# AndreiBarsan/DynSLAM

Hardware: AMD Instinct MI355X
Metric: frames/sec TSDF integrate+raycast (KITTI 1242x375, 5mm voxels); HBM GB/s vs peak (higher is better)
Workload: dtype f32; 1 GPU; configs[1]: static map only, synthetic KITTI-like street 1242x375, preset 5mm (voxel 0.005 m, mu 0.02 m), frames 5..2062 of a 2063-frame sequence, one volume per GPU; visible_blocks_last_frame=122661, allocated_blocks=8388608, status=3, decay=False, swap=False, instances=0

## Files before the change

### __graft_entry__.py

```python
import os
import subprocess
import sys

ROOT = os.path.dirname(os.path.abspath(__file__))
CSRC = os.path.join(ROOT, "dynslam_amd", "csrc")
HIP_LIB = os.path.join(CSRC, "libdsr_hip.so")
HIP_SOURCES = ["dsr_engine.hip", "dsr_view.hip", "dsr_exchange.hip", "dsr_hostio.hip", "dsr_profile.hip", "dsr_track.hip",
               "dsr_eval.hip", "dsr_snapshot.hip", "dsr_merge.hip"]
HIP_HEADERS = ["dsr_internal.h", "dsr_device.h", "k_alloc.h", "k_small.h", "k_batch.h", "k_composite.h", "k_decay.h", "k_edges.h", "k_integrate.h",
               "k_raycast.h", "k_swap.h", "k_mesh.h", "mc_tables.h", "k_track.h", "k_batch_track.h", "dsr_math.h", "k_eval.h",
               "k_batch_gc.h", "k_snapshot.h", "k_mesh_complete.h", "k_merge.h"]
HIPCC_COMPILE_FLAGS = ["--offload-arch=gfx950", "-O3", "-std=c++17", "-fPIC", "-ffp-contract=off", "-fno-slp-vectorize",
                       "-fno-fast-math", "-Wall", "-Wno-unused-function"]
HIPCC_FLAGS = HIPCC_COMPILE_FLAGS + ["-shared"]


def _stale(target, deps):
    if not os.path.exists(target):
        return True
    t = os.path.getmtime(target)
    return any(os.path.getmtime(d) > t for d in deps)


def build_hip(force=False):
    srcs = [os.path.join(CSRC, s) for s in HIP_SOURCES]
    deps = srcs + [os.path.join(CSRC, h) for h in HIP_HEADERS] + [os.path.join(ROOT, "include", h) for h in ("dsr.h", "dsr_track.h", "dsr_eval.h", "dsr_gc.h", "dsr_snapshot.h", "dsr_mesh.h")]
# ... 97 lines not shown
```

### dynslam_amd/csrc/dsr_engine.hip

```cpp
#include <sched.h>

#include "dsr_internal.h"
#include "dsr_math.h"
using namespace dsr_internal;
#include "k_alloc.h"
#include "k_composite.h"
#include "k_decay.h"
#include "k_integrate.h"
#include "k_raycast.h"
#include "k_swap.h"
#include "k_mesh.h"
#include "k_mesh_complete.h"
#include "k_small.h"
#include "k_batch.h"
#include "k_batch_gc.h"
#include "../../include/dsr_track.h"
#include "../../include/dsr_gc.h"
#include "../../include/dsr_mesh.h"

extern "C" {
int dsri_batch_flush(dsr_batch *b);
bool dsri_batch_is_live(dsr_batch *b);
void dsri_batch_drop_deferred(dsr_batch *b);
}

namespace dsr_internal {
std::atomic<int> g_enginesOnDevice[64];
}
// ... 22 lines not shown
bool m4_inv(const Mat4 &in, Mat4 &out) { return dsr_math::m4_inv(in.m, out.m); }

}


namespace {

void prof_resolve(dsr_engine *e) {
  if (e->profPending.empty()) return;
  if (e->viewStream) (void)hipStreamSynchronize(e->viewStream);
  (void)hipStreamSynchronize(e->stream);
  if (e->sideStream) (void)hipStreamSynchronize(e->sideStream);
  if (e->device >= 0 && e->device < 64 && g_ioStream[e->device]) (void)hipStreamSynchronize(g_ioStream[e->device]);
  for (auto &p : e->profPending) {
    float ms = 0.0f;
    if (hipEventElapsedTime(&ms, p.a, p.b) == hipSuccess) { e->profRecs[p.rec].ms += ms; e->profRecs[p.rec].launches++; }
    e->eventPool.push_back(p.a); e->eventPool.push_back(p.b);
  }
  e->profPending.clear();
}

FrameP make_frame_params(const dsr_engine *e, const Mat4 &M, const Mat4 &invM, const float proj[4]) {
  FrameP p;
  memset(&p, 0, sizeof p);
  p.M = M; p.invM = invM;
  p.M_rgb = m4_mul(e->calibInv, M);
  p.proj = make_float4(proj[0], proj[1], proj[2], proj[3]);
  p.proj_rgb = make_float4(e->calib.rgb.fx, e->calib.rgb.fy, e->calib.rgb.cx, e->calib.rgb.cy);
  p.mu = e->s.mu; p.voxelSize = e->s.voxel_size;
  p.vfMin = e->s.view_frustum_min; p.vfMax = e->s.view_frustum_max;
  p.W = e->W; p.H = e->H; p.Wr = e->Wr; p.Hr = e->Hr;
// ... 74 lines not shown
    if (e->upPin[k]) (void)hipHostFree(e->upPin[k]);
    if (e->upSlotFree[k]) (void)hipEventDestroy(e->upSlotFree[k]);
  }
  F(e->upDev); F(e->pvDev); F(e->xferRgb); F(e->xferDepth);
  F(e->rgbAlt); F(e->depthAlt);
  for (hipEvent_t ev : {e->evAltFree, e->evFusionRead}) if (ev) (void)hipEventDestroy(ev);
  if (e->viewStream && e->ownsViewStream) (void)hipStreamDestroy(e->viewStream);
  if (e->pvPin) (void)hipHostFree(e->pvPin);
  if (e->statusHost) (void)hipHostFree(e->statusHost);
  for (hipEvent_t ev : {e->evUploaded, e->evIngested, e->evView, e->evViewRead}) if (ev) (void)hipEventDestroy(ev);
  if (e->xEvent) (void)hipEventDestroy(e->xEvent);
  if (e->xEvent2) (void)hipEventDestroy(e->xEvent2);
  if (e->orderEvent) (void)hipEventDestroy(e->orderEvent);
  for (auto &p : e->profPending) { (void)hipEventDestroy(p.a); (void)hipEventDestroy(p.b); }
  for (auto ev : e->eventPool) (void)hipEventDestroy(ev);
  if (e->evList) (void)hipEventDestroy(e->evList);
  if (e->evExpected) (void)hipEventDestroy(e->evExpected);
  if (e->sideStream) (void)hipStreamDestroy(e->sideStream);
  if (e->stream && e->ownsStream) (void)hipStreamDestroy(e->stream);
}

int expected_depths(dsr_engine *e, RenderStateDev &rs, const FrameP &p);

int allocate_scene(dsr_engine *e) {
  e->sceneVersion++;
  e->noVisibleValid = false;
  e->listVersion++;
  float proj[4]; depth_proj(e, proj);
  FrameP p = make_frame_params(e, e->M_d, e->invM_d, proj);
  RenderStateDev &rs = e->live;
// ... 25 lines not shown
         (const float *)e->depth, rs.visType, 0, 0);
  LAUNCH(e, "scan_tiles", k_scan_tile_sums, dim3(1), dim3(1024), allocTile, e->numTilesE, e->scene, (int)SCAN_ALLOC, 0);
  LAUNCH(e, "alloc_commit", k_alloc_commit, dim3(e->numTilesE), dim3(kTileThreads), p, e->scene, allocTile, e->allocWork);
  LAUNCH(e, "alloc_apply", k_alloc_apply, dim3(256), dim3(256), p, e->scene, (const float *)e->depth,
         (const int4 *)e->allocWork, rs.visType);
  LAUNCH(e, "visible_count", k_visible_count<false>, dim3(e->numTilesE), dim3(kTileThreads), p, e->scene, rs.visType, e->tileSums);
  LAUNCH(e, "scan_tiles", k_scan_tile_sums, dim3(1), dim3(1024), e->tileSums, e->numTilesE, e->scene,
         (int)SCAN_VISIBLE_LIVE, e->noBlocks);
  if (e->statusDev) e->statusSeq++;
  LAUNCH(e, "visible_write", k_visible_write, dim3(e->numTilesE), dim3(kTileThreads), e->E, (const uint8_t *)rs.visType,
         (const int2 *)e->tileSums, rs.visibleIDs, e->noBlocks, e->scene, (int)e->s.use_swapping, rs.visBlocks, e->statusDev,
         e->statusSeq);
  HIP_TRY(hipGetLastError());
  { int st = after_fusion(e); if (st) return st; }
  e->liveExp.valid = false;
  if (e->overlapExpected && (e->device >= 64 || g_enginesOnDevice[e->device].load(std::memory_order_relaxed) <= 1)) {
    HIP_TRY(hipEventRecord(e->evList, e->stream));
    HIP_TRY(hipStreamWaitEvent(e->sideStream, e->evList, 0));
    {
      StreamSwap sw(e, e->sideStream);
      int st = expected_depths(e, rs, p);
      if (st) return st;
    }
    HIP_TRY(hipEventRecord(e->evExpected, e->sideStream));
    e->sidePending = true;
    e->liveExp.valid = true; e->liveExp.onSide = true; e->liveExp.version = e->listVersion; e->liveExp.M = e->M_d;
    memcpy(e->liveExp.proj, proj, sizeof proj);
  }
  return DSR_OK;
}

int integrate_scene(dsr_engine *e) {
  e->sceneVersion++;
  float proj[4]; depth_proj(e, proj);
  FrameP p = make_frame_params(e, e->M_d, e->invM_d, proj);
  const bool plain = !p.depthWeighting && !p.stopAtMaxW && e->shortDivMuExact;
  { int st = before_fusion(e); if (st) return st; }
#define LAUNCH_INTEGRATE(A, B, VOX, OCC)                                                                     \
  LAUNCH(e, "integrate", (k_integrate<A, B, VOX, OCC, true>), dim3(e->gridIntegrate), dim3(256), p, e->scene, \
         (const float *)e->depth, (const uchar4 *)e->rgb, (const int4 *)e->live.visBlocks, e->integrateStats)
#define LAUNCH_INTEGRATE_V(VOX, OCC)                                                                         \
  do {                                                                                                       \
    if (p.rgbSame) { if (plain) LAUNCH_INTEGRATE(true, true, VOX, OCC); else LAUNCH_INTEGRATE(true, false, VOX, OCC); } \
    else { if (plain) LAUNCH_INTEGRATE(false, true, VOX, OCC); else LAUNCH_INTEGRATE(false, false, VOX, OCC); }         \
  } while (0)
  LAUNCH_INTEGRATE_V(8, 7);
#undef LAUNCH_INTEGRATE_V
#undef LAUNCH_INTEGRATE
  HIP_TRY(hipGetLastError());
  return after_fusion(e);
}

int expected_depths(dsr_engine *e, RenderStateDev &rs, const FrameP &p) {
  const int mw = (e->W + 7) / 8, mh = (e->H + 7) / 8;
  if (e->smallVolume && (size_t)mw * mh * sizeof(int2) <= 64 * 1024) {
    ProfScope _ps(e, "expected_depth");
    hipLaunchKernelGGL(k_expected_depth_one, dim3(1), dim3(1024), (size_t)mw * mh * sizeof(int2), e->stream, p, e->scene,
                       (const int4 *)rs.visBlocks, rs.ctrIdx, reinterpret_cast<int2 *>(rs.minmax),
                       rs.ctrIdx == CTR_NO_VISIBLE_LIVE ? 1 : 0, rs.rayBox);
    return DSR_OK;
  }
// ... 2 lines not shown
  const size_t ldsBytes = (size_t)mw * mh * sizeof(int2);
  if (ldsBytes <= 64 * 1024) {
    ProfScope _ps(e, "expected_depth");
    hipLaunchKernelGGL(k_expected_depth_lds, dim3(e->gridExpected), dim3(1024), ldsBytes, e->stream, p, e->scene,
                       (const int4 *)rs.visBlocks, rs.ctrIdx, reinterpret_cast<int2 *>(rs.minmax));
  } else {
    LAUNCH(e, "expected_depth", k_expected_depth, dim3(1024), dim3(256), p, e->scene, (const int4 *)rs.visBlocks,
           rs.ctrIdx, reinterpret_cast<int2 *>(rs.minmax));
  }
  return DSR_OK;
}

int launch_raycast(dsr_engine *e, const char *name, const FrameP &p, RenderStateDev &rs) {
  dim3 g(div_up(e->W, 16), div_up(e->H, 16));
  if (rs.rayBox) LAUNCH(e, name, k_raycast_box, g, dim3(256), p, e->scene, rs.ctrIdx, (const float2 *)rs.minmax, rs.raycastResult, rs.rayBox);
  else LAUNCH(e, name, k_raycast, g, dim3(256), p, e->scene, rs.ctrIdx, (const float2 *)rs.minmax, rs.raycastResult);
  return DSR_OK;
}

bool pair_render_default() {
  static const bool on = !(getenv("DSR_PAIR_RENDER") && atoi(getenv("DSR_PAIR_RENDER")) == 0);
  return on;
}
int launch_icp_maps(dsr_engine *e, const FrameP &p) {
  RenderStateDev &rs = e->live;
  dim3 g(div_up(e->W, 16), div_up(e->H, 16));
  if (rs.rayBox) LAUNCH(e, "icp_maps", k_icp_maps_box, g, dim3(256), p, e->scene, (const float4 *)rs.raycastResult, e->pointsMap,
                        e->normalsMap, rs.raycastImage, (const int32_t *)rs.rayBox);
  else LAUNCH(e, "icp_maps", k_icp_maps, g, dim3(256), p, e->scene, (const float4 *)rs.raycastResult, e->pointsMap,
              e->normalsMap, rs.raycastImage);
  return DSR_OK;
// ... 224 lines not shown
  if (s.view_pipeline < DSR_VIEW_PIPELINE_AUTO || s.view_pipeline > DSR_VIEW_PIPELINE_SHARED) { delete e; return fail(DSR_E_ARG, "bad view_pipeline"); }
  const int pvMode = s.view_pipeline == DSR_VIEW_PIPELINE_OFF ? 0 : s.view_pipeline == DSR_VIEW_PIPELINE_PER_ENGINE ? 1
                     : s.view_pipeline == DSR_VIEW_PIPELINE_SHARED ? 3
                     : getenv("DSR_PIPELINED_VIEW") ? atoi(getenv("DSR_PIPELINED_VIEW")) : (s.sync_status ? 3 : 0);
  auto shared_stream = [&](hipStream_t *table) -> hipStream_t {
    if (e->device < 0 || e->device >= 64) return nullptr;
    std::lock_guard<std::mutex> lock(g_ioMutex);
    if (!table[e->device] && create_stream(&table[e->device]) != hipSuccess) table[e->device] = nullptr;
    return table[e->device];
  };
  if (pvMode == 3 && s.sdf_local_block_num <= 16384 && (e->stream = shared_stream(g_sharedViewStream))) e->ownsStream = false;
  else if (pvMode >= 2 && s.sdf_local_block_num <= 16384 && (e->stream = shared_stream(g_sharedSmallStream))) e->ownsStream = false;
  else if (create_stream(&e->stream) != hipSuccess) { delete e; return fail(DSR_E_DEVICE, "hipStreamCreate failed"); }
  e->overlapExpected = s.sdf_local_block_num >= (1 << 20);
  if (const char *ov = getenv("DSR_OVERLAP_EXPECTED")) e->overlapExpected = atoi(ov) != 0;
  if (e->overlapExpected &&
      (hipStreamCreateWithFlags(&e->sideStream, hipStreamNonBlocking) != hipSuccess ||
       hipEventCreateWithFlags(&e->evList, order_event_flags()) != hipSuccess ||
       hipEventCreateWithFlags(&e->evExpected, order_event_flags()) != hipSuccess)) { free_all(e); delete e; return fail(DSR_E_DEVICE, "side stream creation failed"); }
  ALLOC(dmalloc(&e->scene.table, (size_t)e->E));
  ALLOC(dmalloc(&e->scene.vba, (size_t)e->noBlocks * kBlockBytes));
  ALLOC(dmalloc(&e->scene.voxelAllocList, (size_t)e->noBlocks));
  ALLOC(dmalloc(&e->scene.excessAllocList, (size_t)e->noExcess));
  ALLOC(dmalloc(&e->scene.ctr, (size_t)CTR_COUNT));
  ALLOC(dmalloc(&e->scene.work, (size_t)WORK_COUNT));
  ALLOC(dmalloc(&e->scene.allocKey, (size_t)e->E));
  ALLOC(dmalloc(&e->scene.allocGrp, (size_t)e->numTilesE * (kTile / 32)));
  ALLOC(dmalloc(&e->scene.allocTile, (size_t)e->numTilesE + 1));
  {
    const int cells = ((e->W + 7) / 8) * ((e->H + 7) / 8);
// ... 13 lines not shown
  }
  ALLOC(dmalloc(&e->allocWork, (size_t)std::min((double)e->noBlocks, (double)e->P * e->maxSteps)));
  const int mw = (e->W + 7) / 8, mh = (e->H + 7) / 8;
  for (RenderStateDev *rs : {&e->live, &e->freeview}) {
    ALLOC(dmalloc(&rs->visibleIDs, (size_t)e->noBlocks));
    ALLOC(dmalloc(&rs->visBlocks, (size_t)e->noBlocks));
    ALLOC(dmalloc(&rs->visType, (size_t)e->E));
    ALLOC(dmalloc(&rs->minmax, (size_t)mw * mh));
    ALLOC(dmalloc(&rs->raycastResult, (size_t)e->P));
    ALLOC(dmalloc(&rs->raycastImage, (size_t)e->P));
    if (e->smallVolume && (size_t)mw * mh * sizeof(int2) <= 64 * 1024 && !(getenv("DSR_RAY_BOX") && atoi(getenv("DSR_RAY_BOX")) == 0))
      ALLOC(dmalloc(&rs->rayBox, (size_t)RB_WORDS));
  }
  ALLOC(dmalloc(&e->live.visibleIDsAlt, (size_t)e->noBlocks));
  ALLOC(dmalloc(&e->live.visBlocksAlt, (size_t)e->noBlocks));
  e->live.ctrIdx = CTR_NO_VISIBLE_LIVE; e->freeview.ctrIdx = CTR_NO_VISIBLE_FREE;
  ALLOC(dmalloc(&e->tileSums, (size_t)e->numTilesMax + 1));
  e->integrateStatsCount = (size_t)e->gridIntegrate * kIntegrateWaves;
  ALLOC(dmalloc(&e->integrateStats, e->integrateStatsCount));
  (void)hipMemsetAsync(e->integrateStats, 0, e->integrateStatsCount * sizeof(uint2), e->stream);
  ALLOC(dmalloc(&e->rgb, (size_t)e->Wr * e->Hr));
  ALLOC(dmalloc(&e->depth, (size_t)e->P));
  ALLOC(dmalloc(&e->depthTmp, (size_t)e->P));
  ALLOC(dmalloc(&e->rawDepth, (size_t)e->P + 4));
  ALLOC(dmalloc(&e->pointsMap, (size_t)e->P));
  ALLOC(dmalloc(&e->normalsMap, (size_t)e->P));
  ALLOC(dmalloc(&e->scene.icpPose, (size_t)kIcpPoseWords));
  ALLOC(dmalloc(&e->freeDepth, (size_t)e->P));
  ALLOC(dmalloc(&e->decayFlags, (size_t)e->noBlocks));
  ALLOC(dmalloc(&e->decayCand, (size_t)e->noBlocks));
// ... 206 lines not shown
    if (status != DSR_OK) {
      (void)hipMemsetAsync(e->scene.ctr + CTR_STATUS, 0, 4, e->stream);
      if (e->statusHost) e->statusHost[1] = DSR_OK;
      return fail(status, status_text(status));
    }
  }
  return DSR_OK;
}

int dsr_prepare(dsr_engine *e) {
  CHECK_E(e);
  if (!e->hasView) return fail(DSR_E_NO_VIEW, "no view yet");
  float proj[4]; depth_proj(e, proj);
  FrameP p = make_frame_params(e, e->M_d, e->invM_d, proj);
  RenderStateDev &rs = e->live;
  if (e->liveExp.valid && e->liveExp.version == e->listVersion && memcmp(e->liveExp.M.m, e->M_d.m, sizeof e->M_d.m) == 0 &&
      memcmp(e->liveExp.proj, proj, sizeof proj) == 0) {
    if (e->liveExp.onSide) {
      HIP_TRY(hipStreamWaitEvent(e->stream, e->evExpected, 0));
      e->sidePending = false;
    }
  } else {
    if (e->sidePending) { HIP_TRY(hipStreamWaitEvent(e->stream, e->evExpected, 0)); e->sidePending = false; }
    e->liveExp.valid = false;
    int st = expected_depths(e, rs, p);
    if (st) return st;
  }
  if (e->pairRender && rs.rayBox) {
    e->trackRender.pending = true;
    e->trackRender.p = p;
    HIP_TRY(hipGetLastError());
    return DSR_OK;
  }
  {
    int st = launch_raycast(e, "raycast", p, rs);
    if (st) return st;
    if ((st = launch_icp_maps(e, p))) return st;
  }
  HIP_TRY(hipGetLastError());
  return DSR_OK;
}

int dsr_decay(dsr_engine *e, int max_weight, int min_age, int force_all_voxels) {
  CHECK_E(e);
  if (min_age < 0) return fail(DSR_E_ARG, "negative min_age");
  e->sceneVersion++;
  e->noVisibleValid = false;
  e->listVersion++;
  if (e->sidePending) { HIP_TRY(hipStreamWaitEvent(e->stream, e->evExpected, 0)); e->sidePending = false; }
// ... 1138 lines not shown
int dsr_dump_visible_list(dsr_engine *e, int freeview, int32_t *ids_out, int32_t *n) {
  CHECK_E(e);
  if (!n) return fail(DSR_E_ARG, "null");
  RenderStateDev &rs = freeview ? e->freeview : e->live;
  int32_t cnt = 0;
  HIP_TRY(hipMemcpyAsync(&cnt, e->scene.ctr + rs.ctrIdx, 4, hipMemcpyDeviceToHost, e->stream));
  HIP_TRY(hipStreamSynchronize(e->stream));
  *n = cnt;
  if (ids_out && cnt > 0) {
    HIP_TRY(hipMemcpyAsync(ids_out, rs.visibleIDs, (size_t)cnt * 4, hipMemcpyDeviceToHost, e->stream));
    HIP_TRY(hipStreamSynchronize(e->stream));
  }
  return DSR_OK;
}

int dsr_dump_visible_types(dsr_engine *e, uint8_t *out) {
  CHECK_E(e);
  if (!out) return fail(DSR_E_ARG, "null");
  HIP_TRY(hipMemcpyAsync(out, e->live.visType, (size_t)e->E, hipMemcpyDeviceToHost, e->stream));
  HIP_TRY(hipStreamSynchronize(e->stream));
  return DSR_OK;
}

int dsr_dump_voxel_blocks(dsr_engine *e, int first_block, int n_blocks, dsr_voxel *out) {
  CHECK_E(e);
  if (!out || first_block < 0 || n_blocks < 0 || (long long)first_block + n_blocks > e->noBlocks) return fail(DSR_E_ARG, "bad block range");
  const int chunk = 16384;
  if (e->aosScratchBlocks < std::min(chunk, n_blocks)) {
    if (e->aosScratch) (void)hipFree(e->aosScratch);
    e->aosScratch = nullptr;
// ... 44 lines not shown
```

### dynslam_amd/csrc/dsr_internal.h

```cpp
#pragma once
#include <hip/hip_runtime.h>

#include <algorithm>
#include <atomic>
#include <cmath>
#include <cstdio>
#include <cstdlib>
#include <cstring>
#include <map>
#include <mutex>
#include <new>
#include <string>
#include <unordered_map>
#include <vector>

#include "dsr_device.h"
#include "../../include/dsr_mesh.h"
#include "../../include/dsr_track.h"

using namespace dsr;

namespace dsr_internal {
std::string &last_error();
inline int fail(int code, const std::string &msg) { last_error() = msg; return code; }
// ... 23 lines not shown
  int ctrIdx = CTR_NO_VISIBLE_LIVE;
};

struct ProfRec { std::string name; double ms = 0; long long launches = 0; };

struct dsr_engine {
  dsr_settings s;
  dsr_calib calib;
  int device = 0;
  hipStream_t stream = nullptr;
  hipStream_t sideStream = nullptr;
  hipEvent_t evList = nullptr, evExpected = nullptr;
  bool overlapExpected = true;
  unsigned long long listVersion = 0;
  struct { bool valid = false; bool onSide = false; unsigned long long version = 0; Mat4 M; float proj[4] = {0, 0, 0, 0}; } liveExp;
  int W = 0, H = 0, Wr = 0, Hr = 0, P = 0;
  int noBuckets = 0, noExcess = 0, E = 0, noBlocks = 0;
  int numTilesE = 0, numTilesB = 0, numTilesMax = 0;
  uint32_t maxSteps = 0;
  int gridPersistent = 2048;
  int gridDecay = 2048;
  int gridIntegrate = 8192;
  bool smallVolume = false;
  bool smallPath = false;
  bool smallLists = false;
  size_t smallLdsBytes = 0;
  int viewBox[4] = {0, 0, 0, 0};
  int blankBox[4] = {0, 0, 0, 0};
  bool blankValid = false;
  int gridExpected = 128;
// ... 84 lines not shown
  hipEvent_t xEvent = nullptr;
  hipEvent_t xEvent2 = nullptr;
  bool xEvent2System = false;
  hipEvent_t orderEvent = nullptr;
  uint8_t *decayFlags = nullptr;

  bool pairRender = false;
  bool rayBoxLive = false;
  struct { bool pending = false; FrameP p; } trackRender;
  struct dsr_batch *ownerBatch = nullptr;
  struct TrackerDev *tracker = nullptr;

  int profiling = 0;
  std::vector<ProfRec> profRecs;
  std::map<std::string, int> profIndex;
  struct Pending { int rec; hipEvent_t a, b; };
  std::vector<Pending> profPending;
  std::vector<hipEvent_t> eventPool;
};

namespace dsr_internal {
inline int set_device(dsr_engine *e) {
  HIP_TRY(hipSetDevice(e->device));
  return DSR_OK;
}
inline hipEvent_t get_event(dsr_engine *e) {
  if (!e->eventPool.empty()) { hipEvent_t ev = e->eventPool.back(); e->eventPool.pop_back(); return ev; }
  hipEvent_t ev = nullptr;
  (void)hipEventCreate(&ev);
  return ev;
}
void prof_resolve_pending(dsr_engine *e);
struct ProfScope {
  dsr_engine *e; int rec = -1; hipEvent_t a = nullptr, b = nullptr;
  ProfScope(dsr_engine *e_, const char *name) : e(e_) {
    if (!e->profiling) return;
    if (e->profiling == 2 && strcmp(name, "integrate") != 0 && strcmp(name, "raycast") != 0 && strcmp(name, "raycast_tail") != 0) return;
    auto it = e->profIndex.find(name);
    if (it == e->profIndex.end()) {
      rec = (int)e->profRecs.size();
      e->profIndex[name] = rec;
      ProfRec r; r.name = name; e->profRecs.push_back(r);
    } else rec = it->second;
    if (e->profPending.size() > 8192) prof_resolve_pending(e);
    a = get_event(e); b = get_event(e);
    (void)hipEventRecord(a, e->stream);
  }
  ~ProfScope() {
    if (rec < 0) return;
    (void)hipEventRecord(b, e->stream);
    e->profPending.push_back({rec, a, b});
  }
};
struct StreamSwap {
  dsr_engine *e; hipStream_t saved;
  StreamSwap(dsr_engine *e_, hipStream_t s) : e(e_), saved(e_->stream) { e->stream = s; }
  ~StreamSwap() { e->stream = saved; }
};
inline int div_up(long long a, long long b) { return (int)((a + b - 1) / b); }
template <class T>
int dmalloc(T **p, size_t n) {
  HIP_TRY(hipMalloc(reinterpret_cast<void **>(p), n * sizeof(T)));
  return DSR_OK;
}
extern std::mutex g_ioMutex;
extern hipStream_t g_ioStream[64];
// ... 32 lines not shown
template <class T>
int device_alloc(T **p, size_t n) {
  HIP_TRY(hipMalloc(reinterpret_cast<void **>(p), n * sizeof(T)));
  return DSR_OK;
}
}
using dsr_internal::host_range_pinned;
using dsr_internal::short_division_exact;

#define LAUNCH(e, name, kernel, grid, block, ...)                                \
  do {                                                                           \
    dsr_internal::ProfScope _ps((e), (name));                                    \
    hipLaunchKernelGGL(kernel, grid, block, 0, (e)->stream, __VA_ARGS__);        \
  } while (0)

#define CHECK_E_NOFLUSH(e)                                  \
  if (!(e)) return fail(DSR_E_ARG, "null engine");          \
  { int _st = dsr_internal::engine_set_device(e); if (_st) return _st; }
#define CHECK_E(e)                                          \
  CHECK_E_NOFLUSH(e)                                        \
  if ((e)->trackRender.pending || (e)->ownerBatch) { int _st = dsr_internal::engine_flush_deferred(e); if (_st) return _st; }
```

### dynslam_amd/csrc/k_batch.h

```cpp
#pragma once
#include "k_integrate.h"
#include "k_small.h"

namespace dsr {

constexpr int kBatchMax = 8;

struct BatchVolP {
  SceneP s;
  float *depth;
  uchar4 *rgb;
  uint8_t *visType;
  int4 *workList;
  int32_t *visibleIDs;
  int4 *visBlocks;
  int2 *minmax;
  float4 *raycastResult;
  uchar4 *raycastImage;
  float4 *pointsMap, *normalsMap;
  uint2 *integrateStats;
  int32_t *fvVisibleIDs;
  int4 *fvVisBlocks;
  int2 *fvMinmax;
  float4 *fvRaycastResult;
// ... 68 lines not shown
__global__ __launch_bounds__(kSmallThreads) void k_batch_small_alloc_visible(const BatchFrames frames,
                                                                             const BatchVolP *__restrict__ vols) {
  const BatchFrameP &f = frames.f[blockIdx.x];
  if (!f.active) return;
  const BatchVolP &v = vols[blockIdx.x];
  small_alloc_visible_body(f.p, v.s, v.depth, v.visType, v.numTiles, v.workList, v.visibleIDs, v.visBlocks, v.noBlocks, v.statusDev,
                           f.publishSeq, v.minmax, v.rayBox, v.lists);
}

template <bool RGB_SAME, bool PLAIN>
__global__ __launch_bounds__(64 * kIntegrateWaves, 7) void k_batch_integrate(const BatchFrames frames,
                                                                             const BatchVolP *__restrict__ vols) {
  const BatchFrameP &f = frames.f[blockIdx.y];
  const BatchVolP &v = vols[blockIdx.y];
  if (!f.active || (int)blockIdx.x >= v.gridIntegrate) return;
  integrate_body<RGB_SAME, PLAIN, 8, true>(f.p, v.s, v.depth, v.rgb, v.visBlocks, v.integrateStats, (int)blockIdx.x, v.gridIntegrate);
}

__global__ __launch_bounds__(256, 8) void k_batch_raycast(const BatchFrames frames, const BatchVolP *__restrict__ vols) {
  const BatchFrameP &f = frames.f[blockIdx.z];
  if (!f.active) return;
  const BatchVolP &v = vols[blockIdx.z];
  if (v.s.ctr[CTR_NO_VISIBLE_LIVE] <= 0) return;
  if (v.rayBox) {
    if (blockIdx.x == 0 && blockIdx.y == 0 && threadIdx.x == 0) raybox_mark_ran(v.rayBox, f.p);
    if (!raybox_tile(v.rayBox, RB_DIRTY, blockIdx.x, blockIdx.y)) return;
  }
  const int lane = threadIdx.x & 63, wave = threadIdx.x >> 6;
  const int x = blockIdx.x * 16 + (wave & 1) * 8 + (lane & 7);
  const int y = blockIdx.y * 16 + (wave >> 1) * 8 + (lane >> 3);
  if (x >= f.p.W || y >= f.p.H) return;
// ... 85 lines not shown
```

### dynslam_amd/csrc/k_integrate.h

```cpp
#pragma once
#include <type_traits>

#include "dsr_device.h"

namespace dsr {

__device__ __forceinline__ float3 bilinear_rgb(const uchar4 *__restrict__ src, float px, float py, int W) {
  const int ix = f2i(floorf(px)), iy = f2i(floorf(py));
  const float dx = px - (float)ix, dy = py - (float)iy;
  const uchar4 a = src[ix + iy * W];
  const uchar4 b = src[(ix + 1) + iy * W];
  const uchar4 c = src[ix + (iy + 1) * W];
  const uchar4 d = src[(ix + 1) + (iy + 1) * W];
  float3 r;
  r.x = ((float)a.x * (1.0f - dx) * (1.0f - dy) + (float)b.x * dx * (1.0f - dy) + (float)c.x * (1.0f - dx) * dy + (float)d.x * dx * dy);
  r.y = ((float)a.y * (1.0f - dx) * (1.0f - dy) + (float)b.y * dx * (1.0f - dy) + (float)c.y * (1.0f - dx) * dy + (float)d.y * dx * dy);
  r.z = ((float)a.z * (1.0f - dx) * (1.0f - dy) + (float)b.z * dx * (1.0f - dy) + (float)c.z * (1.0f - dx) * dy + (float)d.z * dx * dy);
  return r;
}

__device__ __forceinline__ int depth_weight(float depth_measure) {
  int w = f2i(10.0f / depth_measure + 0.5f);
  return w < 1 ? 1 : w;
}
// ... 22 lines not shown
}
template <int VOX>
__device__ __forceinline__ void store_planes(uint8_t *blk, int vox0, const LanePlanes<VOX> &r) {
  if (VOX == 8) {
    *reinterpret_cast<uint4 *>(blk + kOffSdf + vox0 * 2) = make_uint4(r.sdf[0], r.sdf[1], r.sdf[VOX / 2 - 2], r.sdf[VOX / 2 - 1]);
    *reinterpret_cast<uint2 *>(blk + kOffWDepth + vox0) = make_uint2(r.wd[0], r.wd[VOX / 4 - 1]);
  } else {
    *reinterpret_cast<uint2 *>(blk + kOffSdf + vox0 * 2) = make_uint2(r.sdf[0], r.sdf[VOX / 2 - 1]);
    *reinterpret_cast<uint32_t *>(blk + kOffWDepth + vox0) = r.wd[0];
  }
}

template <bool RGB_SAME, bool PLAIN, int VOX, bool XLDS>
__device__ __forceinline__ void integrate_body(const FrameP &p, const SceneP &s, const float *__restrict__ depth,
                                               const uchar4 *__restrict__ rgb, const int4 *__restrict__ visBlocks,
                                               uint2 *__restrict__ waveStats, const int blockId, const int numBlocks) {
  constexpr int kTasksPerBlock = 8 / VOX;
  constexpr int kVoxPerTask = kBlockSize3 / kTasksPerBlock;
  constexpr int kPendCap = 64 + kVoxPerTask;
  __shared__ uint32_t s_pend[kIntegrateWaves][kPendCap];
  __shared__ float s_rcpW[257];
  __shared__ float4 s_xprod[XLDS ? kIntegrateWaves : 1][8];
  static_assert(!XLDS || VOX == 8, "the x positions are wave-uniform only when a lane owns a whole x row");
  for (int i = threadIdx.x; i < 257; i += 64 * kIntegrateWaves) s_rcpW[i] = 1.0f / (float)(i > 0 ? i : 1);
  __syncthreads();

  const int noVisible = s.ctr[CTR_NO_VISIBLE_LIVE];
  const int noTasks = noVisible * kTasksPerBlock;
  if (blockId == 0 && threadIdx.x == 0) atomicAdd(&s.work[WORK_V_INTEGRATED], (unsigned long long)noVisible);
  const bool stopAtMaxW = PLAIN ? false : (p.stopAtMaxW != 0);
  const bool depthWeighting = PLAIN ? false : (p.depthWeighting != 0);
  const int lane = threadIdx.x & 63;
  const int wave = __builtin_amdgcn_readfirstlane(threadIdx.x >> 6);
  const int stride = numBlocks * kIntegrateWaves;
  const Mat4 &Mr = RGB_SAME ? p.M : p.M_rgb;
  const float4 projr = RGB_SAME ? p.proj : p.proj_rgb;
  const int Wc = RGB_SAME ? p.W : p.Wr, Hc = RGB_SAME ? p.H : p.Hr;
  uint32_t *pend = s_pend[wave];
  const int t0 = blockId * kIntegrateWaves + wave;
  int maxWv = p.maxW;
  asm volatile("" : "+v"(maxWv));

// ... 213 lines not shown
      colour_pass(nPend, 64);
    }
  }
  if (nPend > 0) colour_pass(0, nPend);
  if (lane == 0 && (statStoreLanes | statColour)) {
    uint2 *slot = waveStats + (blockId * kIntegrateWaves + wave);
    const uint2 old = *slot;
    *slot = make_uint2(old.x + statStoreLanes, old.y + statColour);
  }
}

template <bool RGB_SAME, bool PLAIN, int VOX, int OCC, bool XLDS = false>
__global__ __launch_bounds__(64 * kIntegrateWaves, OCC) void k_integrate(FrameP p, SceneP s, const float *__restrict__ depth,
                                                                         const uchar4 *__restrict__ rgb,
                                                                         const int4 *__restrict__ visBlocks,
                                                                         uint2 *__restrict__ waveStats) {
  integrate_body<RGB_SAME, PLAIN, VOX, XLDS>(p, s, depth, rgb, visBlocks, waveStats, (int)blockIdx.x, (int)gridDim.x);
}

}
```

### dynslam_amd/csrc/k_raycast.h

```cpp
#pragma once
#include "dsr_device.h"

namespace dsr {


struct VoxCache {
  int bx, by, bz;
  int ptr;
};
__host__ __device__ __forceinline__ void cache_init(VoxCache &c) { c.bx = c.by = c.bz = 0x7fffffff; c.ptr = -1; }

__host__ __device__ __forceinline__ int find_block(const SceneP &s, const FrameP &p, int x, int y, int z, int &linearIdx,
                                          VoxCache &cache) {
  const int bx = x >> 3, by = y >> 3, bz = z >> 3;
  linearIdx = (x & 7) + ((y & 7) << 3) + ((z & 7) << 6);
  if (bx == cache.bx && by == cache.by && bz == cache.bz) return cache.ptr;
  uint32_t hashIdx = hash_index(bx, by, bz, p.hashMask);
  while (true) {
    dsr_hash_entry he = load_entry(s.table, hashIdx);
    if (he.pos[0] == bx && he.pos[1] == by && he.pos[2] == bz && he.ptr >= 0) {
      cache.bx = bx; cache.by = by; cache.bz = bz; cache.ptr = he.ptr;
      return he.ptr;
    }
    if (he.offset < 1) break;
// ... 455 lines not shown
  out.x = rx; out.y = ry; out.z = rz;
  return out;
}

template <class Ops>
__host__ __device__ __forceinline__ float4 cast_ray(const FrameP &p, const SceneP &s, int x, int y, float2 mm RC_STAT(, RcStats &st)) {
  RayState r;
  ray_setup<Ops>(p, x, y, mm, r);
  VoxCache cache; cache_init(cache);
  VoxCache cache2; cache_init(cache2);
  const float sdfValue = ray_march<Ops>(p, s, r, cache, cache2 RC_STAT(, st));
  return ray_finish<Ops>(p, s, r, sdfValue, cache, cache2);
}

__global__ __launch_bounds__(256, 8) void k_raycast(FrameP p, SceneP s, int ctrIdx, const float2 *__restrict__ minmax,
                                                 float4 *__restrict__ raycastResult) {
  if (s.ctr[ctrIdx] <= 0 && ctrIdx == CTR_NO_VISIBLE_LIVE) return;
  const int lane = threadIdx.x & 63, wave = threadIdx.x >> 6;
  const int wgx = blockIdx.x, wgy = blockIdx.y;
  const int x = wgx * 16 + (wave & 1) * 8 + (lane & 7);
  const int y = wgy * 16 + (wave >> 1) * 8 + (lane >> 3);
  if (x >= p.W || y >= p.H) return;
  const int mw = (p.W + kMinmaxSubsample - 1) / kMinmaxSubsample;
  const float2 mm = minmax[(x >> 3) + (y >> 3) * mw];
#ifdef DSR_RAYCAST_STATS
  const unsigned long long t0 = wall_clock64();
  RcStats st;
  raycastResult[x + y * p.W] = cast_ray<DeviceOps>(p, s, x, y, mm, st);
  const unsigned long long t1 = wall_clock64();
  unsigned own = st.nLook + st.nVox + st.nBand, iter = st.nIter, look = st.nLook, sumIter = st.nIter;
  for (int d = 1; d < 64; d <<= 1) {
    own = max(own, (unsigned)__shfl_xor((int)own, d)); iter = max(iter, (unsigned)__shfl_xor((int)iter, d));
    st.wLook = max(st.wLook, (unsigned)__shfl_xor((int)st.wLook, d)); st.wBand = max(st.wBand, (unsigned)__shfl_xor((int)st.wBand, d));
    st.wHead = max(st.wHead, (unsigned)__shfl_xor((int)st.wHead, d)); st.wChain = max(st.wChain, (unsigned)__shfl_xor((int)st.wChain, d));
// ... 374 lines not shown
```

### dynslam_amd/engine.py

```python
import ctypes as C
import os

import numpy as np

from . import _capi
from ._capi import (BLOCK_SIZE3, DSR_E_OUT_OF_BLOCKS, DSR_OK, Calib, KernelTime,
                    Settings, Stats)

HASH_ENTRY_DTYPE = np.dtype([("pos", "<i2", (3,)), ("pad", "<i2"), ("offset", "<i4"), ("ptr", "<i4")])
VOXEL_DTYPE = np.dtype([("sdf", "<i2"), ("w_depth", "u1"), ("clr", "u1", (3,)), ("w_color", "u1"), ("pad", "u1")])
assert HASH_ENTRY_DTYPE.itemsize == 16 and VOXEL_DTYPE.itemsize == 8

_HERE = os.path.dirname(os.path.abspath(__file__))
HIP_LIB_PATH = os.environ.get("DSR_HIP_LIB") or os.path.join(_HERE, "csrc", "libdsr_hip.so")

_hip_api = None


class DsrError(RuntimeError):
    def __init__(self, status, message):
        super().__init__(f"dsr status {status}: {message}")
        self.status = status


# ... 524 lines not shown
        st = Stats()
        self._check(self.api.get_stats(self._h, C.byref(st)))
        return st

    def dump_hash_table(self):
        out = np.empty(self.no_total_entries, HASH_ENTRY_DTYPE)
        self._check(self.api.dump_hash_table(self._h, _ptr(out)))
        return out

    def dump_visible_list(self, freeview=False):
        ids = np.empty(self.no_blocks, np.int32)
        n = C.c_int32(0)
        self._check(self.api.dump_visible_list(self._h, int(freeview), _ptr(ids), C.byref(n)))
        return ids[: n.value].copy()

    def dump_visible_types(self):
        out = np.empty(self.no_total_entries, np.uint8)
        self._check(self.api.dump_visible_types(self._h, _ptr(out)))
        return out

    def dump_voxel_blocks(self, first_block=0, n_blocks=None):
        if n_blocks is None:
            n_blocks = self.no_blocks - first_block
        out = np.empty((n_blocks, BLOCK_SIZE3), VOXEL_DTYPE)
        self._check(self.api.dump_voxel_blocks(self._h, int(first_block), int(n_blocks), _ptr(out)))
        return out

    def dump_allocation_lists(self):
        v = np.empty(self.no_blocks, np.int32)
        x = np.empty(self.settings.excess_list_size, np.int32)
# ... 323 lines not shown
```

Baseline: 3698 frames/s.

## Partition visible blocks into screen bands to overlap integrate with raycast

Adds a kernel that sorts visible blocks into screen-column bands by their projected footprint. Integration runs once per band with an event after each, and the raycast for each band starts on a side stream as soon as its band is integrated, so raycast overlaps the remaining integration. Blocks that span more than two bands go to band 0 so they are finished first. This costs an extra partition kernel, more launches and events, and a conservative footprint test that must be correct or the output changes. It is enabled by default only for large volumes (at least 2^20 blocks) without swapping.

After: 3171 frames/s. -14.2%, worse.

```diff
diff --git a/__graft_entry__.py b/__graft_entry__.py
--- a/__graft_entry__.py
+++ b/__graft_entry__.py
@@ -9,7 +9,7 @@
                "dsr_eval.hip", "dsr_snapshot.hip", "dsr_merge.hip"]
 HIP_HEADERS = ["dsr_internal.h", "dsr_device.h", "k_alloc.h", "k_small.h", "k_batch.h", "k_composite.h", "k_decay.h", "k_edges.h", "k_integrate.h",
                "k_raycast.h", "k_swap.h", "k_mesh.h", "mc_tables.h", "k_track.h", "k_batch_track.h", "dsr_math.h", "k_eval.h",
-               "k_batch_gc.h", "k_snapshot.h", "k_mesh_complete.h", "k_merge.h"]
+               "k_batch_gc.h", "k_snapshot.h", "k_mesh_complete.h", "k_merge.h", "k_bands.h"]
 HIPCC_COMPILE_FLAGS = ["--offload-arch=gfx950", "-O3", "-std=c++17", "-fPIC", "-ffp-contract=off", "-fno-slp-vectorize",
                        "-fno-fast-math", "-Wall", "-Wno-unused-function"]
 HIPCC_FLAGS = HIPCC_COMPILE_FLAGS + ["-shared"]
diff --git a/dynslam_amd/csrc/dsr_engine.hip b/dynslam_amd/csrc/dsr_engine.hip
--- a/dynslam_amd/csrc/dsr_engine.hip
+++ b/dynslam_amd/csrc/dsr_engine.hip
@@ -12,6 +12,7 @@
 #include "k_mesh.h"
 #include "k_mesh_complete.h"
 #include "k_small.h"
+#include "k_bands.h"
 #include "k_batch.h"
 #include "k_batch_gc.h"
 #include "../../include/dsr_track.h"
@@ -64,7 +65,7 @@
   if (e->device >= 0 && e->device < 64 && g_ioStream[e->device]) (void)hipStreamSynchronize(g_ioStream[e->device]);
   for (auto &p : e->profPending) {
     float ms = 0.0f;
-    if (hipEventElapsedTime(&ms, p.a, p.b) == hipSuccess) { e->profRecs[p.rec].ms += ms; e->profRecs[p.rec].launches++; }
+    if (hipEventElapsedTime(&ms, p.a, p.b) == hipSuccess) { e->profRecs[p.rec].ms += ms; e->profRecs[p.rec].launches += p.launches; }
     e->eventPool.push_back(p.a); e->eventPool.push_back(p.b);
   }
   e->profPending.clear();
@@ -169,6 +170,9 @@
   if (e->orderEvent) (void)hipEventDestroy(e->orderEvent);
   for (auto &p : e->profPending) { (void)hipEventDestroy(p.a); (void)hipEventDestroy(p.b); }
   for (auto ev : e->eventPool) (void)hipEventDestroy(ev);
+  F(e->bandTable); F(e->bandCtr); F(e->visBlocksBanded);
+  for (hipEvent_t ev : e->evBand) if (ev) (void)hipEventDestroy(ev);
+  if (e->evSideRay) (void)hipEventDestroy(e->evSideRay);
   if (e->evList) (void)hipEventDestroy(e->evList);
   if (e->evExpected) (void)hipEventDestroy(e->evExpected);
   if (e->sideStream) (void)hipStreamDestroy(e->sideStream);
@@ -224,6 +228,7 @@
   HIP_TRY(hipGetLastError());
   { int st = after_fusion(e); if (st) return st; }
   e->liveExp.valid = false;
+  e->bands.valid = false; e->bands.integrated = false;
   if (e->overlapExpected && (e->device >= 64 || g_enginesOnDevice[e->device].load(std::memory_order_relaxed) <= 1)) {
     HIP_TRY(hipEventRecord(e->evList, e->stream));
     HIP_TRY(hipStreamWaitEvent(e->sideStream, e->evList, 0));
@@ -236,6 +241,14 @@
     e->sidePending = true;
     e->liveExp.valid = true; e->liveExp.onSide = true; e->liveExp.version = e->listVersion; e->liveExp.M = e->M_d;
     memcpy(e->liveExp.proj, proj, sizeof proj);
+    if (e->overlapRaycast) {
+      LAUNCH(e, "band_partition", k_band_partition, dim3(std::min(1024, std::max(1, div_up(e->noBlocks, kBandChunk)))),
+             dim3(kBandThreads), p, e->scene, (const int4 *)rs.visBlocks, e->noBlocks, (const int32_t *)e->bandTable,
+             e->visBlocksBanded, e->bandCtr);
+      HIP_TRY(hipGetLastError());
+      e->bands.valid = true; e->bands.integrated = false; e->bands.version = e->listVersion; e->bands.M = e->M_d;
+      memcpy(e->bands.proj, proj, sizeof proj);
+    }
   }
   return DSR_OK;
 }
@@ -246,15 +259,30 @@
   FrameP p = make_frame_params(e, e->M_d, e->invM_d, proj);
   const bool plain = !p.depthWeighting && !p.stopAtMaxW && e->shortDivMuExact;
   { int st = before_fusion(e); if (st) return st; }
-#define LAUNCH_INTEGRATE(A, B, VOX, OCC)                                                                     \
-  LAUNCH(e, "integrate", (k_integrate<A, B, VOX, OCC, true>), dim3(e->gridIntegrate), dim3(256), p, e->scene, \
-         (const float *)e->depth, (const uchar4 *)e->rgb, (const int4 *)e->live.visBlocks, e->integrateStats)
+#define LAUNCH_INTEGRATE(A, B, VOX, OCC)                                                                                   \
+  LAUNCH_N(e, "integrate", countLaunch, (k_integrate<A, B, VOX, OCC, true>), dim3(e->gridIntegrate), dim3(256), p, e->scene, \
+           (const float *)e->depth, (const uchar4 *)e->rgb, (const int4 *)stream16, e->integrateStats, range)
 #define LAUNCH_INTEGRATE_V(VOX, OCC)                                                                         \
   do {                                                                                                       \
     if (p.rgbSame) { if (plain) LAUNCH_INTEGRATE(true, true, VOX, OCC); else LAUNCH_INTEGRATE(true, false, VOX, OCC); } \
     else { if (plain) LAUNCH_INTEGRATE(false, true, VOX, OCC); else LAUNCH_INTEGRATE(false, false, VOX, OCC); }         \
   } while (0)
-  LAUNCH_INTEGRATE_V(8, 7);
+  const int4 *stream16 = e->live.visBlocks;
+  const int32_t *range = nullptr;
+  int countLaunch = 1;
+  if (e->overlapRaycast && e->bands.valid && e->bands.version == e->listVersion) {
+    stream16 = e->visBlocksBanded;
+    for (int b = 0; b < e->numBands; ++b) {
+      range = e->bandCtr + BAND_RANGE + 2 * b;
+      countLaunch = b == 0 ? 1 : 0;
+      LAUNCH_INTEGRATE_V(8, 7);
+      HIP_TRY(hipEventRecord(e->evBand[b], e->stream));
+    }
+    e->bands.integrated = true; e->bands.sceneVersion = e->sceneVersion;
+  } else {
+    e->bands.integrated = false;
+    LAUNCH_INTEGRATE_V(8, 7);
+  }
 #undef LAUNCH_INTEGRATE_V
 #undef LAUNCH_INTEGRATE
   HIP_TRY(hipGetLastError());
@@ -287,7 +315,14 @@
 int launch_raycast(dsr_engine *e, const char *name, const FrameP &p, RenderStateDev &rs) {
   dim3 g(div_up(e->W, 16), div_up(e->H, 16));
   if (rs.rayBox) LAUNCH(e, name, k_raycast_box, g, dim3(256), p, e->scene, rs.ctrIdx, (const float2 *)rs.minmax, rs.raycastResult, rs.rayBox);
-  else LAUNCH(e, name, k_raycast, g, dim3(256), p, e->scene, rs.ctrIdx, (const float2 *)rs.minmax, rs.raycastResult);
+  else LAUNCH(e, name, k_raycast, g, dim3(256), p, e->scene, rs.ctrIdx, (const float2 *)rs.minmax, rs.raycastResult, 0);
+  return DSR_OK;
+}
+int launch_raycast_band(dsr_engine *e, const FrameP &p, RenderStateDev &rs, int b, int countLaunch) {
+  const int x0 = e->bandBounds[b], nx = e->bandBounds[b + 1] - x0;
+  if (nx <= 0) return DSR_OK;
+  LAUNCH_N(e, "raycast", countLaunch, k_raycast, dim3(nx, div_up(e->H, 16)), dim3(256), p, e->scene, rs.ctrIdx,
+           (const float2 *)rs.minmax, rs.raycastResult, x0);
   return DSR_OK;
 }
 
@@ -542,6 +577,11 @@
   else if (create_stream(&e->stream) != hipSuccess) { delete e; return fail(DSR_E_DEVICE, "hipStreamCreate failed"); }
   e->overlapExpected = s.sdf_local_block_num >= (1 << 20);
   if (const char *ov = getenv("DSR_OVERLAP_EXPECTED")) e->overlapExpected = atoi(ov) != 0;
+  int overlapRaycastMode = 1;
+  if (const char *orc = getenv("DSR_OVERLAP_RAYCAST")) overlapRaycastMode = atoi(orc);
+  if (overlapRaycastMode == 2 && !getenv("DSR_OVERLAP_EXPECTED")) e->overlapExpected = true;
+  e->overlapRaycast = overlapRaycastMode != 0 && e->overlapExpected && !s.use_swapping && !e->smallVolume &&
+                      (overlapRaycastMode == 2 || s.sdf_local_block_num >= (1 << 20));
   if (e->overlapExpected &&
       (hipStreamCreateWithFlags(&e->sideStream, hipStreamNonBlocking) != hipSuccess ||
        hipEventCreateWithFlags(&e->evList, order_event_flags()) != hipSuccess ||
@@ -585,6 +625,23 @@
   }
   ALLOC(dmalloc(&e->live.visibleIDsAlt, (size_t)e->noBlocks));
   ALLOC(dmalloc(&e->live.visBlocksAlt, (size_t)e->noBlocks));
+  if (e->overlapRaycast) {
+    static_assert(dsr_engine::kMaxRayBands == kMaxBands, "one constant");
+    e->numBands = 2;
+    if (const char *nb = getenv("DSR_RAYCAST_BANDS")) e->numBands = std::min(kMaxBands, std::max(2, atoi(nb)));
+    const int tilesX = div_up(e->W, 16);
+    int32_t tab[kBandTableWords] = {};
+    tab[0] = e->numBands;
+    for (int b = 0; b <= e->numBands; ++b) tab[1 + b] = e->bandBounds[b] = (int)((long long)tilesX * b / e->numBands);
+    ALLOC(dmalloc(&e->bandTable, (size_t)kBandTableWords));
+    ALLOC(dmalloc(&e->bandCtr, (size_t)kBandCtrWords));
+    ALLOC(dmalloc(&e->visBlocksBanded, (size_t)e->noBlocks * (e->numBands > 2 ? 2 : 1)));
+    if (hipMemcpy(e->bandTable, tab, sizeof tab, hipMemcpyHostToDevice) != hipSuccess ||
+        hipMemset(e->bandCtr, 0, kBandCtrWords * sizeof(int32_t)) != hipSuccess) { free_all(e); delete e; return fail(DSR_E_DEVICE, "band table upload failed"); }
+    for (int b = 0; b < e->numBands; ++b)
+      if (hipEventCreateWithFlags(&e->evBand[b], order_event_flags()) != hipSuccess) { free_all(e); delete e; return fail(DSR_E_DEVICE, "band event creation failed"); }
+    if (hipEventCreateWithFlags(&e->evSideRay, order_event_flags()) != hipSuccess) { free_all(e); delete e; return fail(DSR_E_DEVICE, "band event creation failed"); }
+  }
   e->live.ctrIdx = CTR_NO_VISIBLE_LIVE; e->freeview.ctrIdx = CTR_NO_VISIBLE_FREE;
   ALLOC(dmalloc(&e->tileSums, (size_t)e->numTilesMax + 1));
   e->integrateStatsCount = (size_t)e->gridIntegrate * kIntegrateWaves;
@@ -821,8 +878,9 @@
   float proj[4]; depth_proj(e, proj);
   FrameP p = make_frame_params(e, e->M_d, e->invM_d, proj);
   RenderStateDev &rs = e->live;
-  if (e->liveExp.valid && e->liveExp.version == e->listVersion && memcmp(e->liveExp.M.m, e->M_d.m, sizeof e->M_d.m) == 0 &&
-      memcmp(e->liveExp.proj, proj, sizeof proj) == 0) {
+  const bool reused = e->liveExp.valid && e->liveExp.version == e->listVersion && memcmp(e->liveExp.M.m, e->M_d.m, sizeof e->M_d.m) == 0 &&
+                      memcmp(e->liveExp.proj, proj, sizeof proj) == 0;
+  if (reused) {
     if (e->liveExp.onSide) {
       HIP_TRY(hipStreamWaitEvent(e->stream, e->evExpected, 0));
       e->sidePending = false;
@@ -839,7 +897,28 @@
     HIP_TRY(hipGetLastError());
     return DSR_OK;
   }
-  {
+  if (reused && e->liveExp.onSide && e->overlapRaycast && !rs.rayBox && e->bands.integrated && e->bands.version == e->listVersion &&
+      e->bands.sceneVersion == e->sceneVersion &&
+      memcmp(e->bands.M.m, e->M_d.m, sizeof e->M_d.m) == 0 && memcmp(e->bands.proj, proj, sizeof proj) == 0) {
+    const int B = e->numBands;
+    int counted = 0;
+    {
+      StreamSwap sw(e, e->sideStream);
+      for (int b = 0; b < B - 1; ++b) {
+        if (e->bandBounds[b + 1] <= e->bandBounds[b]) continue;
+        HIP_TRY(hipStreamWaitEvent(e->sideStream, e->evBand[b], 0));
+        int st = launch_raycast_band(e, p, rs, b, counted ? 0 : 1);
+        if (st) return st;
+        counted = 1;
+      }
+      HIP_TRY(hipEventRecord(e->evSideRay, e->sideStream));
+    }
+    int st = launch_raycast_band(e, p, rs, B - 1, counted ? 0 : 1);
+    if (st) return st;
+    HIP_TRY(hipStreamWaitEvent(e->stream, e->evSideRay, 0));
+    if ((st = launch_icp_maps(e, p))) return st;
+    e->bands.integrated = false;
+  } else {
     int st = launch_raycast(e, "raycast", p, rs);
     if (st) return st;
     if ((st = launch_icp_maps(e, p))) return st;
@@ -2008,6 +2087,23 @@
   return DSR_OK;
 }
 
+int dsr_dump_band_partition(dsr_engine *e, int32_t *info, int32_t *live_out, int32_t *banded_out) {
+  CHECK_E(e);
+  if (!info) return fail(DSR_E_ARG, "null");
+  memset(info, 0, 16 * sizeof(int32_t));
+  HIP_TRY(hipMemcpyAsync(info + 1, e->scene.ctr + CTR_NO_VISIBLE_LIVE, 4, hipMemcpyDeviceToHost, e->stream));
+  HIP_TRY(hipStreamSynchronize(e->stream));
+  if (!e->overlapRaycast || !e->bands.valid || e->bands.version != e->listVersion) return DSR_OK;
+  info[0] = e->numBands;
+  for (int b = 0; b <= e->numBands; ++b) info[2 + b] = e->bandBounds[b];
+  HIP_TRY(hipMemcpyAsync(info + 8, e->bandCtr + BAND_RANGE, 2 * kMaxBands * sizeof(int32_t), hipMemcpyDeviceToHost, e->stream));
+  const size_t n = (size_t)std::max(0, std::min(info[1], e->noBlocks));
+  if (live_out && n) HIP_TRY(hipMemcpyAsync(live_out, e->live.visBlocks, n * 16, hipMemcpyDeviceToHost, e->stream));
+  if (banded_out && n) HIP_TRY(hipMemcpyAsync(banded_out, e->visBlocksBanded, n * (e->numBands > 2 ? 2 : 1) * 16, hipMemcpyDeviceToHost, e->stream));
+  HIP_TRY(hipStreamSynchronize(e->stream));
+  return DSR_OK;
+}
+
 int dsr_dump_visible_types(dsr_engine *e, uint8_t *out) {
   CHECK_E(e);
   if (!out) return fail(DSR_E_ARG, "null");
diff --git a/dynslam_amd/csrc/dsr_internal.h b/dynslam_amd/csrc/dsr_internal.h
--- a/dynslam_amd/csrc/dsr_internal.h
+++ b/dynslam_amd/csrc/dsr_internal.h
@@ -61,6 +61,14 @@
   bool overlapExpected = true;
   unsigned long long listVersion = 0;
   struct { bool valid = false; bool onSide = false; unsigned long long version = 0; Mat4 M; float proj[4] = {0, 0, 0, 0}; } liveExp;
+  static constexpr int kMaxRayBands = 4;
+  bool overlapRaycast = false;
+  int numBands = 2;
+  int bandBounds[kMaxRayBands + 1] = {0, 0, 0, 0, 0};
+  int32_t *bandTable = nullptr, *bandCtr = nullptr;
+  int4 *visBlocksBanded = nullptr;
+  hipEvent_t evBand[kMaxRayBands] = {nullptr, nullptr, nullptr, nullptr}, evSideRay = nullptr;
+  struct { bool valid = false; bool integrated = false; unsigned long long version = 0, sceneVersion = 0; Mat4 M; float proj[4] = {0, 0, 0, 0}; } bands;
   int W = 0, H = 0, Wr = 0, Hr = 0, P = 0;
   int noBuckets = 0, noExcess = 0, E = 0, noBlocks = 0;
   int numTilesE = 0, numTilesB = 0, numTilesMax = 0;
@@ -175,7 +183,7 @@
   int profiling = 0;
   std::vector<ProfRec> profRecs;
   std::map<std::string, int> profIndex;
-  struct Pending { int rec; hipEvent_t a, b; };
+  struct Pending { int rec; hipEvent_t a, b; int launches; };
   std::vector<Pending> profPending;
   std::vector<hipEvent_t> eventPool;
 };
@@ -194,7 +202,8 @@
 void prof_resolve_pending(dsr_engine *e);
 struct ProfScope {
   dsr_engine *e; int rec = -1; hipEvent_t a = nullptr, b = nullptr;
-  ProfScope(dsr_engine *e_, const char *name) : e(e_) {
+  int launches;
+  ProfScope(dsr_engine *e_, const char *name, int launches_ = 1) : e(e_), launches(launches_) {
     if (!e->profiling) return;
     if (e->profiling == 2 && strcmp(name, "integrate") != 0 && strcmp(name, "raycast") != 0 && strcmp(name, "raycast_tail") != 0) return;
     auto it = e->profIndex.find(name);
@@ -210,7 +219,7 @@
   ~ProfScope() {
     if (rec < 0) return;
     (void)hipEventRecord(b, e->stream);
-    e->profPending.push_back({rec, a, b});
+    e->profPending.push_back({rec, a, b, launches});
   }
 };
 struct StreamSwap {
@@ -273,6 +282,12 @@
     hipLaunchKernelGGL(kernel, grid, block, 0, (e)->stream, __VA_ARGS__);        \
   } while (0)
 
+#define LAUNCH_N(e, name, count, kernel, grid, block, ...)                       \
+  do {                                                                           \
+    dsr_internal::ProfScope _ps((e), (name), (count));                           \
+    hipLaunchKernelGGL(kernel, grid, block, 0, (e)->stream, __VA_ARGS__);        \
+  } while (0)
+
 #define CHECK_E_NOFLUSH(e)                                  \
   if (!(e)) return fail(DSR_E_ARG, "null engine");          \
   { int _st = dsr_internal::engine_set_device(e); if (_st) return _st; }
diff --git a/dynslam_amd/csrc/k_bands.h b/dynslam_amd/csrc/k_bands.h
--- /dev/null
+++ b/dynslam_amd/csrc/k_bands.h
@@ -0,0 +1,100 @@
+#pragma once
+#include "dsr_device.h"
+
+namespace dsr {
+
+constexpr int kMaxBands = 4;
+constexpr int kBandEnlargeVoxels = 2;
+constexpr float kBandNearZ = 1e-10f;
+constexpr int kBandTableWords = 2 + kMaxBands;
+constexpr int BAND_TICKET = kMaxBands, BAND_RANGE = 8, kBandCtrWords = BAND_RANGE + 2 * kMaxBands;
+constexpr int kBandChunk = 4096, kBandThreads = 256;
+
+__host__ __device__ __forceinline__ int band_of_tile(const int32_t *tab, int tile) {
+  const int B = tab[0];
+  int b = 0;
+  while (b < B - 1 && tab[2 + b] <= tile) ++b;
+  return b;
+}
+
+template <int ENLARGE>
+__host__ __device__ __forceinline__ int band_launch_index(const short pos[3], const Mat4 &M, const float4 &proj, float voxelSize,
+                                                          int W, const int32_t *tab) {
+  const float lo = -(float)ENLARGE, hi = (float)(kBlockSize + ENLARGE);
+  float xmin = 3.0e38f, xmax = -3.0e38f;
+  for (int c = 0; c < 8; ++c) {
+    const float x = ((float)(pos[0] * kBlockSize) + ((c & 1) ? hi : lo)) * voxelSize;
+    const float y = ((float)(pos[1] * kBlockSize) + ((c & 2) ? hi : lo)) * voxelSize;
+    const float z = ((float)(pos[2] * kBlockSize) + ((c & 4) ? hi : lo)) * voxelSize;
+    const float3 q = mat_mul3(M, x, y, z, 1.0f);
+    if (!(q.z >= kBandNearZ)) return 0;
+    const float u = proj.x * q.x / q.z + proj.z;
+    if (!(u == u)) return 0;
+    xmin = u < xmin ? u : xmin;
+    xmax = u > xmax ? u : xmax;
+  }
+  xmin -= 1.0f; xmax += 1.0f;
+  const float wLast = (float)(W - 1);
+  const float a = fminf(fmaxf(floorf(xmin), 0.0f), wLast), b = fminf(fmaxf(ceilf(xmax), 0.0f), wLast);
+  const int bandLo = band_of_tile(tab, (int)a >> 4), bandHi = band_of_tile(tab, (int)b >> 4);
+  return (bandHi - bandLo > 1) ? 0 : bandLo;
+}
+
+__device__ __forceinline__ int band_slot(int b, int n, int rank) {
+  return (b & 1) ? ((b + 1) >> 1) * n - 1 - rank : (b >> 1) * n + rank;
+}
+
+#ifdef __HIPCC__
+__global__ __launch_bounds__(kBandThreads) void k_band_partition(FrameP p, SceneP s, const int4 *__restrict__ visBlocks, int capacity,
+                                                               const int32_t *__restrict__ tab, int4 *__restrict__ banded,
+                                                               int32_t *__restrict__ bandCtr) {
+  constexpr int kItems = kBandChunk / kBandThreads;
+  __shared__ int cnt[kMaxBands], base[kMaxBands];
+  __shared__ int32_t tabLds[kBandTableWords];
+  int n = s.ctr[CTR_NO_VISIBLE_LIVE];
+  n = n < capacity ? n : capacity;
+  if (threadIdx.x < kBandTableWords) tabLds[threadIdx.x] = tab[threadIdx.x];
+  const int B = tab[0];
+  for (int c0 = blockIdx.x * kBandChunk; c0 < n; c0 += gridDim.x * kBandChunk) {
+    if (threadIdx.x < kMaxBands) cnt[threadIdx.x] = 0;
+    __syncthreads();
+    uint32_t lr[kItems];
+#pragma unroll
+    for (int k = 0; k < kItems; ++k) {
+      const int i = c0 + k * kBandThreads + threadIdx.x;
+      lr[k] = 0;
+      if (i < n) {
+        const dsr_hash_entry he = entry_of_record(visBlocks[i]);
+        const int li = band_launch_index<kBandEnlargeVoxels>(he.pos, p.M, p.proj, p.voxelSize, p.W, tabLds);
+        lr[k] = ((uint32_t)li << 16) | (uint32_t)atomicAdd(&cnt[li], 1);
+      }
+    }
+    __syncthreads();
+    if ((int)threadIdx.x < B && cnt[threadIdx.x] > 0) base[threadIdx.x] = atomicAdd(&bandCtr[threadIdx.x], cnt[threadIdx.x]);
+    __syncthreads();
+#pragma unroll
+    for (int k = 0; k < kItems; ++k) {
+      const int i = c0 + k * kBandThreads + threadIdx.x;
+      if (i < n) {
+        const int li = (int)(lr[k] >> 16);
+        banded[band_slot(li, n, base[li] + (int)(lr[k] & 0xffffu))] = visBlocks[i];
+      }
+    }
+    __syncthreads();
+  }
+  if (threadIdx.x == 0) {
+    const int ticket = atomicAdd(&bandCtr[BAND_TICKET], 1);
+    if (ticket == (int)gridDim.x - 1) {
+      for (int b = 0; b < kMaxBands; ++b) {
+        const int c = atomicExch(&bandCtr[b], 0);
+        const int start = (b & 1) ? ((b + 1) >> 1) * n - c : (b >> 1) * n;
+        bandCtr[BAND_RANGE + 2 * b] = start;
+        bandCtr[BAND_RANGE + 2 * b + 1] = start + c;
+      }
+      atomicExch(&bandCtr[BAND_TICKET], 0);
+    }
+  }
+}
+#endif
+
+}
diff --git a/dynslam_amd/csrc/k_batch.h b/dynslam_amd/csrc/k_batch.h
--- a/dynslam_amd/csrc/k_batch.h
+++ b/dynslam_amd/csrc/k_batch.h
@@ -106,7 +106,8 @@
   const BatchFrameP &f = frames.f[blockIdx.y];
   const BatchVolP &v = vols[blockIdx.y];
   if (!f.active || (int)blockIdx.x >= v.gridIntegrate) return;
-  integrate_body<RGB_SAME, PLAIN, 8, true>(f.p, v.s, v.depth, v.rgb, v.visBlocks, v.integrateStats, (int)blockIdx.x, v.gridIntegrate);
+  integrate_body<RGB_SAME, PLAIN, 8, true>(f.p, v.s, v.depth, v.rgb, v.visBlocks, v.integrateStats, (int)blockIdx.x, v.gridIntegrate,
+                                           v.s.ctr[CTR_NO_VISIBLE_LIVE]);
 }
 
 __global__ __launch_bounds__(256, 8) void k_batch_raycast(const BatchFrames frames, const BatchVolP *__restrict__ vols) {
diff --git a/dynslam_amd/csrc/k_integrate.h b/dynslam_amd/csrc/k_integrate.h
--- a/dynslam_amd/csrc/k_integrate.h
+++ b/dynslam_amd/csrc/k_integrate.h
@@ -60,7 +60,8 @@
 template <bool RGB_SAME, bool PLAIN, int VOX, bool XLDS>
 __device__ __forceinline__ void integrate_body(const FrameP &p, const SceneP &s, const float *__restrict__ depth,
                                                const uchar4 *__restrict__ rgb, const int4 *__restrict__ visBlocks,
-                                               uint2 *__restrict__ waveStats, const int blockId, const int numBlocks) {
+                                               uint2 *__restrict__ waveStats, const int blockId, const int numBlocks,
+                                               const int noVisible) {
   constexpr int kTasksPerBlock = 8 / VOX;
   constexpr int kVoxPerTask = kBlockSize3 / kTasksPerBlock;
   constexpr int kPendCap = 64 + kVoxPerTask;
@@ -71,7 +72,6 @@
   for (int i = threadIdx.x; i < 257; i += 64 * kIntegrateWaves) s_rcpW[i] = 1.0f / (float)(i > 0 ? i : 1);
   __syncthreads();
 
-  const int noVisible = s.ctr[CTR_NO_VISIBLE_LIVE];
   const int noTasks = noVisible * kTasksPerBlock;
   if (blockId == 0 && threadIdx.x == 0) atomicAdd(&s.work[WORK_V_INTEGRATED], (unsigned long long)noVisible);
   const bool stopAtMaxW = PLAIN ? false : (p.stopAtMaxW != 0);
@@ -315,8 +315,12 @@
 __global__ __launch_bounds__(64 * kIntegrateWaves, OCC) void k_integrate(FrameP p, SceneP s, const float *__restrict__ depth,
                                                                          const uchar4 *__restrict__ rgb,
                                                                          const int4 *__restrict__ visBlocks,
-                                                                         uint2 *__restrict__ waveStats) {
-  integrate_body<RGB_SAME, PLAIN, VOX, XLDS>(p, s, depth, rgb, visBlocks, waveStats, (int)blockIdx.x, (int)gridDim.x);
-}
-
-}
+                                                                         uint2 *__restrict__ waveStats,
+                                                                         const int32_t *__restrict__ range) {
+  const int start = range ? range[0] : 0;
+  const int end = range ? range[1] : s.ctr[CTR_NO_VISIBLE_LIVE];
+  integrate_body<RGB_SAME, PLAIN, VOX, XLDS>(p, s, depth, rgb, visBlocks + start, waveStats, (int)blockIdx.x, (int)gridDim.x,
+                                             end - start);
+}
+
+}
diff --git a/dynslam_amd/csrc/k_raycast.h b/dynslam_amd/csrc/k_raycast.h
--- a/dynslam_amd/csrc/k_raycast.h
+++ b/dynslam_amd/csrc/k_raycast.h
@@ -493,10 +493,10 @@
 }
 
 __global__ __launch_bounds__(256, 8) void k_raycast(FrameP p, SceneP s, int ctrIdx, const float2 *__restrict__ minmax,
-                                                 float4 *__restrict__ raycastResult) {
+                                                 float4 *__restrict__ raycastResult, int wgx0) {
   if (s.ctr[ctrIdx] <= 0 && ctrIdx == CTR_NO_VISIBLE_LIVE) return;
   const int lane = threadIdx.x & 63, wave = threadIdx.x >> 6;
-  const int wgx = blockIdx.x, wgy = blockIdx.y;
+  const int wgx = blockIdx.x + wgx0, wgy = blockIdx.y;
   const int x = wgx * 16 + (wave & 1) * 8 + (lane & 7);
   const int y = wgy * 16 + (wave >> 1) * 8 + (lane >> 3);
   if (x >= p.W || y >= p.H) return;
diff --git a/dynslam_amd/engine.py b/dynslam_amd/engine.py
--- a/dynslam_amd/engine.py
+++ b/dynslam_amd/engine.py
@@ -562,6 +562,17 @@
         self._check(self.api.dump_visible_list(self._h, int(freeview), _ptr(ids), C.byref(n)))
         return ids[: n.value].copy()
 
+    def dump_band_partition(self):
+        fn = self.api.lib.dsr_dump_band_partition
+        fn.restype, fn.argtypes = C.c_int, [C.c_void_p] * 4
+        info = np.zeros(16, np.int32)
+        self._check(fn(self._h, _ptr(info), None, None))
+        n, slots = int(info[1]), int(info[1]) * (2 if info[0] > 2 else 1)
+        live, banded = np.zeros((n, 4), np.int32), np.zeros((slots, 4), np.int32)
+        if info[0] > 0 and n > 0:
+            self._check(fn(self._h, _ptr(info), _ptr(live), _ptr(banded)))
+        return info, live, banded
+
     def dump_visible_types(self):
         out = np.empty(self.no_total_entries, np.uint8)
         self._check(self.api.dump_visible_types(self._h, _ptr(out)))
```
